# linnanwang/FastGen

Hardware: AMD Instinct MI355X
Metric: images/sec at 4-step distilled (DMD2) sampling (higher is better)
Workload: dtype fp32 (tensors, accumulate) with split-bf16 x3 MFMA conv products; 1 GPU; EDM CIFAR-10 32x32 SongUNet (55.7M params) DMD2 4-step 'sde' sampling, batch=512 per GPU; global_batch=512, sample_steps=4, parallelism=replicas x1 (no data-path collective), graph=True

## Files before the change

### fastgen_amd/csrc/conv_ws3.hip

```cpp
#include "common.h"
#include "conv.h"

namespace {

constexpr int X3_NTHR = 768;
constexpr int X3_KC = 32;
constexpr int X3_PA = 16;
constexpr int X3_PLANE = 3072;
constexpr int X3_ABUF = 8 * X3_PLANE;
constexpr int X3_RING = 4;
constexpr int X3_HOFF = 128 * 512;
constexpr int X3_LDS = X3_HOFF + X3_RING * X3_ABUF;
constexpr int X3_TAPB = 2048;

template <int LOGW>
struct X3Geom {
    static constexpr int W = 1 << LOGW;
    static constexpr int TW = 16, TH = 8;
    static constexpr int IPT = LOGW == 3 ? 2 : 1;
    static constexpr int TCOLS = LOGW == 3 ? 1 : W / TW;
    static constexpr int TPI = LOGW == 3 ? 1 : (W / TH) * TCOLS;
    static constexpr int HW_ = LOGW == 3 ? 2 * W + 3 : TW + 2, HH_ = TH + 2;
    static constexpr int HALO_PIX = HW_ * HH_;
    static constexpr int RS = HW_ * X3_PA;
    static_assert(HALO_PIX * X3_PA <= X3_PLANE && HALO_PIX <= 192, "one halo plane; three producer passes of 64 pixels");
};

__device__ __forceinline__ void x3_barrier() {
    asm volatile("s_waitcnt lgkmcnt(0)\n\ts_barrier" ::: "memory");
}

struct X3Frag {
    bf16x8 hi, lo;
};

template <int RES, int LOGW, int PRO>
__global__ __launch_bounds__(X3_NTHR) void conv3_x3ws_kernel(const ConvArgs a, const int ntiles) {
    using G = X3Geom<LOGW>;
    constexpr bool SUB = RES == RES_SUBPIX;
    constexpr int NTAP = SUB ? 4 : 9;
    constexpr int RN = SUB ? 4 : 3;
    constexpr int NQ = 4 * NTAP;
    constexpr int X3_STEPB = NTAP * X3_TAPB;
    extern __shared__ __attribute__((aligned(16))) char smem[];
    char* const hbuf = smem;
    char* const ring = smem + X3_HOFF;

    const int tid = threadIdx.x;
    const int lane = tid & 63;
    const int wave = __builtin_amdgcn_readfirstlane(tid >> 6);
    const int Cin = a.C1 + a.C2;
    const int nchunk = Cin / X3_KC;
    const int G8 = (int)gridDim.x >> 3;
    const int wg = ((gridDim.x & 7) == 0) ? ((int)blockIdx.x & 7) * G8 + ((int)blockIdx.x >> 3) : (int)blockIdx.x;
    const int gstride = (int)gridDim.x;
    const int my_tiles = (ntiles - wg + gstride - 1) / gstride;
    const int S = my_tiles * nchunk;
    const int NSTEP = S + 3;
    const int H = SUB ? a.Hs : a.H;

    if (wave < 8) {
        const int grp = wave >> 2, wl = wave & 3;
        const int col = lane & 15, g4 = lane >> 4;
        const size_t wstride = (size_t)nchunk * NTAP * 1024;
        const __amdgpu_buffer_rsrc_t wrs = __builtin_amdgcn_make_buffer_rsrc(
            const_cast<__bf16*>(reinterpret_cast<const __bf16*>(a.wpack_ws) + (size_t)(grp * 8 + wl * 2) * wstride), 0, 0x7fffffff,
            0x00020000);
        const int wvoff = lane * 16;
        const int wsb = (int)(wstride * 2);
        const int wphb = SUB ? 16 * wsb : 0;
        int tcur = wg;
        auto load_w = [&](int byte_off) -> X3Frag {
            X3Frag f;
            f.hi = __builtin_bit_cast(bf16x8, __builtin_amdgcn_raw_buffer_load_b128(wrs, wvoff, byte_off, 0));
            f.lo = __builtin_bit_cast(bf16x8, __builtin_amdgcn_raw_buffer_load_b128(wrs, wvoff, byte_off + 1024, 0));
            return f;
        };
        X3Frag wq[RN][2];
#pragma unroll
        for (int j = 0; j < RN; ++j)
#pragma unroll
            for (int nt = 0; nt < 2; ++nt) wq[j][nt] = load_w((tcur & 3) * wphb + nt * wsb + j * X3_TAPB);

        f32x4 acc[8][2];
#pragma unroll
        for (int m = 0; m < 8; ++m)
#pragma unroll
            for (int nt = 0; nt < 2; ++nt) acc[m][nt] = f32x4{0.f, 0.f, 0.f, 0.f};

        const int lane_off = g4 * X3_PLANE + (col + ((G::IPT == 2 && col >= 8) ? 1 : 0)) * X3_PA;
        const int dl0 = col * 512 + ((8 * wl + ((g4) ^ (col & 7))) << 4);
        const int dl1 = col * 512 + ((8 * wl + ((4 + g4) ^ (col & 7))) << 4);

        x3_barrier();
        int c = 0;
        for (int s = 0; s < NSTEP; ++s) {
            const int ls = s - 2 * grp;
            if (ls >= 0 && ls < S) {
                const char* abase = ring + (ls & 3) * X3_ABUF + lane_off + (SUB ? ((tcur >> 1) & 1) * G::RS + (tcur & 1) * X3_PA : 0);
                const int cn = (c + 1 == nchunk) ? 0 : c + 1;
                const int tnext = cn == 0 ? tcur + gstride : tcur;
                const int wcur = (tcur & 3) * wphb + c * X3_STEPB;
                const int wnxt = (ls + 1 < S) ? (tnext & 3) * wphb + cn * X3_STEPB : wcur;
                auto read_x = [&](int q, X3Frag (&xf)[2]) {
                    const int tap = q >> 2, m0 = 2 * (q & 3);
                    const int off = ((SUB ? tap >> 1 : tap / 3) + m0) * G::RS + (SUB ? tap & 1 : tap % 3) * X3_PA;
#pragma unroll
                    for (int m = 0; m < 2; ++m) {
                        xf[m].hi = *reinterpret_cast<const bf16x8*>(abase + off + m * G::RS);
                        xf[m].lo = *reinterpret_cast<const bf16x8*>(abase + off + m * G::RS + 4 * X3_PLANE);
                    }
                };
                auto mma12 = [&](int q, const X3Frag (&xf)[2]) {
                    const int tap = q >> 2, m0 = 2 * (q & 3);
                    const X3Frag(&wf)[2] = wq[tap % RN];
#pragma unroll
                    for (int m = 0; m < 2; ++m)
#pragma unroll
                        for (int nt = 0; nt < 2; ++nt)
                            acc[m0 + m][nt] = __builtin_amdgcn_mfma_f32_16x16x32_bf16(wf[nt].hi, xf[m].lo, acc[m0 + m][nt], 0, 0, 0);
#pragma unroll
                    for (int m = 0; m < 2; ++m)
#pragma unroll
                        for (int nt = 0; nt < 2; ++nt)
                            acc[m0 + m][nt] = __builtin_amdgcn_mfma_f32_16x16x32_bf16(wf[nt].lo, xf[m].hi, acc[m0 + m][nt], 0, 0, 0);
#pragma unroll
                    for (int m = 0; m < 2; ++m)
#pragma unroll
                        for (int nt = 0; nt < 2; ++nt)
                            acc[m0 + m][nt] = __builtin_amdgcn_mfma_f32_16x16x32_bf16(wf[nt].hi, xf[m].hi, acc[m0 + m][nt], 0, 0, 0);
                    if ((q & 3) != 3) return;
                    const int pn = (tap + RN < NTAP) ? wcur + (tap + RN) * X3_TAPB : wnxt + (tap + RN - NTAP) * X3_TAPB;
#pragma unroll
                    for (int nt = 0; nt < 2; ++nt) wq[tap % RN][nt] = load_w(pn + nt * wsb);
                };
                X3Frag x0[2], x1[2];
                read_x(0, x0);
#pragma unroll
                for (int q = 0; q < NQ; q += 2) {
                    read_x(q + 1, x1);
                    __builtin_amdgcn_sched_barrier(0);
                    mma12(q, x0);
                    __builtin_amdgcn_sched_barrier(0);
                    if (q + 2 < NQ) read_x(q + 2, x0);
                    __builtin_amdgcn_sched_barrier(0);
                    mma12(q + 1, x1);
                    __builtin_amdgcn_sched_barrier(0);
                }
                if (c + 1 == nchunk) {
#pragma unroll
                    for (int m = 0; m < 8; ++m) {
                        *reinterpret_cast<f32x4*>(hbuf + m * 8192 + dl0) = acc[m][0];
                        *reinterpret_cast<f32x4*>(hbuf + m * 8192 + dl1) = acc[m][1];
                        acc[m][0] = f32x4{0.f, 0.f, 0.f, 0.f};
                        acc[m][1] = f32x4{0.f, 0.f, 0.f, 0.f};
                    }
                }
                c = cn;
                tcur = tnext;
            }
            x3_barrier();
        }
        return;
    }

    const int ptid = tid - 512;
    const int pw = wave - 8;
    const int oct = ptid & 3;
    const float* src1 = reinterpret_cast<const float*>(a.src1);
    const float* src2 = reinterpret_cast<const float*>(a.src2);
    int hdy[3], hdx[3], hlds[3];
    bool third;
    const int pslot = ptid >> 2;
    const int pimg = (G::IPT == 2 && pslot >= 30) ? 1 : 0;
#pragma unroll
    for (int i = 0; i < 3; ++i) {
        int hy, hx;
        if (G::IPT == 2) {
            const int l = pimg ? min(pslot - 30 + 34 * i, 99) : pslot + 30 * i;
            hy = pimg ? l / 10 : l / 9;
            hx = pimg ? 9 + (l - hy * 10) : l - hy * 9;
            third = pimg ? pslot - 30 + 68 < 100 : true;
        } else {
            const int hq = min(pslot + 64 * i, G::HALO_PIX - 1);
            hy = hq / G::HW_;
            hx = hq - hy * G::HW_;
            third = pslot + 128 < G::HALO_PIX;
        }
        hdy[i] = hy - 1;
        hdx[i] = hx - 1 - pimg * (G::W + 1);
        hlds[i] = oct * X3_PLANE + hy * G::RS + hx * X3_PA;
    }

    auto tile_coord = [&](int t, int& n, int& slot, int& row0, int& col0) {
        if (SUB) t >>= 2;
        n = t * G::IPT / G::TPI;
        slot = t - n * G::TPI / G::IPT;
        row0 = (slot / G::TCOLS) * G::TH;
        col0 = (slot % G::TCOLS) * G::TW;
    };

    struct Staged {
        f32x4 raw[3][2];
        float2 ab[8];
    };
    unsigned off1[3], off2[3];
    bool valid[3];
    const float2* abn = a.ab;
    auto tile_setup = [&](int t) __attribute__((always_inline)) {
        int n, slot, row0, col0;
        tile_coord(t, n, slot, row0, col0);
        bool in_batch = true;
        if (G::IPT == 2) {
            n += pimg;
            in_batch = n < a.B;
            n = min(n, a.B - 1);
        }
#pragma unroll
        for (int i = 0; i < 3; ++i) {
            const int y = row0 + hdy[i], x = col0 + hdx[i];
            valid[i] = (y >= 0) && (y < H) && (x >= 0) && (x < G::W) && (i < 2 || third) && in_batch;
            const int yc = min(max(y, 0), H - 1), xc = min(max(x, 0), G::W - 1);
            const int sy = (RES == RES_UP) ? (yc >> 1) : yc, sx = (RES == RES_UP) ? (xc >> 1) : xc;
            const unsigned pix = (unsigned)((n * a.Hs + sy) * a.Ws + sx);
            off1[i] = (pix * (unsigned)a.C1 + oct * 8) * 4u;
            off2[i] = (pix * (unsigned)a.C2 + oct * 8) * 4u;
        }
        abn = a.ab + (size_t)n * Cin;
    };
    auto stage_load = [&](Staged& st, int t, int c32) __attribute__((always_inline)) {
        if (c32 == 0) tile_setup(t);
        const bool first = c32 * X3_KC < a.C1;
        const char* base = first ? reinterpret_cast<const char*>(src1) + c32 * (X3_KC * 4)
                                 : reinterpret_cast<const char*>(src2) + (c32 * X3_KC - a.C1) * 4;
#pragma unroll
        for (int i = 0; i < 3; ++i) {
            const char* p = base + (first ? off1[i] : off2[i]);
            st.raw[i][0] = *reinterpret_cast<const f32x4*>(p);
            st.raw[i][1] = *reinterpret_cast<const f32x4*>(p + 16);
        }
        if (PRO == PRO_NONE) return;
        const float2* p = abn + c32 * X3_KC + oct * 8;
#pragma unroll
        for (int j = 0; j < 8; j += 2) {
            const f32x4 q = *reinterpret_cast<const f32x4*>(p + j);
            st.ab[j] = make_float2(q[0], q[1]);
            st.ab[j + 1] = make_float2(q[2], q[3]);
        }
    };
    auto stage_store = [&](const Staged& st, char* abuf) __attribute__((always_inline)) {
#pragma unroll
        for (int i = 0; i < 3; ++i) {
            float v[8];
#pragma unroll
            for (int j = 0; j < 8; ++j) {
                v[j] = st.raw[i][j >> 2][j & 3];
                if (PRO != PRO_NONE) v[j] = silu_f<true>(fmaf(v[j], st.ab[j].x, st.ab[j].y));
            }
            bf16x8 hi, lo;
            split8(v, hi, lo);
            typedef __attribute__((ext_vector_type(4))) unsigned u32x4;
            u32x4 wh = __builtin_bit_cast(u32x4, hi), wl_ = __builtin_bit_cast(u32x4, lo);
#pragma unroll
            for (int j = 0; j < 4; ++j) {
                wh[j] = valid[i] ? wh[j] : 0u;
                wl_[j] = valid[i] ? wl_[j] : 0u;
            }
            if (i < 2 || third) {
                *reinterpret_cast<u32x4*>(abuf + hlds[i]) = wh;
                *reinterpret_cast<u32x4*>(abuf + hlds[i] + 4 * X3_PLANE) = wl_;
            }
        }
    };

    const int chq = lane & 31, psub = lane >> 5;
    float* const out = reinterpret_cast<float*>(a.out);
    const float* const resid = reinterpret_cast<const float*>(a.resid);
    const bool has_resid = __builtin_amdgcn_readfirstlane(resid != nullptr);
    auto retire_half = [&](int t, int half) __attribute__((always_inline)) {
        int n, slot, row0, col0;
        tile_coord(t, n, slot, row0, col0);
        const int co = half * 128 + chq * 4;
        const int nimg = G::IPT == 2 ? min(2, a.B - n) : 1;
        f32x4 radd[G::IPT];
#pragma unroll
        for (int k = 0; k < G::IPT; ++k) {
            radd[k] = f32x4{0.f, 0.f, 0.f, 0.f};
            if (a.bias) radd[k] = *reinterpret_cast<const f32x4*>(a.bias + co);
            const int nk = G::IPT == 2 ? min(n + k, a.B - 1) : n;
            if (a.temb) radd[k] += *reinterpret_cast<const f32x4*>(a.temb + (size_t)nk * a.temb_stride + co);
            radd[k] *= a.scale;
        }
        constexpr int OW = SUB ? 2 * G::W : G::W, OST = SUB ? 2 : 1;
        const int ph = t & 3;
        const size_t tb = SUB ? (((size_t)n * (2 * H) + 2 * row0 + (ph >> 1)) * OW + 2 * col0 + (ph & 1)) * 256 + co
                              : (((size_t)n * H + row0) * G::W + col0) * 256 + co;
        const int rs = (SUB || G::IPT == 2) ? 0 : a.rshift;
        const size_t rtb = (SUB || G::IPT == 2) ? tb : (((size_t)n * (H >> rs) + (row0 >> rs)) * (G::W >> rs) + (col0 >> rs)) * 256 + co;
        float ssum[G::IPT] = {}, ssq[G::IPT] = {};
#pragma unroll 1
        for (int grp8 = 0; grp8 < 2; ++grp8) {
            f32x4 rr[8], dv[8];
            unsigned go[8];
#pragma unroll
            for (int j = 0; j < 8; ++j) {
                const int px = pw * 32 + 2 * (grp8 * 8 + j) + psub;
                unsigned rgo;
                if (G::IPT == 2) {
                    go[j] = (unsigned)((((j >> 2) * OW + OST * (px >> 4)) * OW + OST * (px & 7)) * 256);
                    rgo = go[j];
                } else {
                    go[j] = (unsigned)((OST * (px >> 4) * OW + OST * (px & 15)) * 256);
                    rgo = SUB ? go[j] : (unsigned)((((px >> 4) >> rs) * (G::W >> rs) + ((px & 15) >> rs)) * 256);
                }
                rr[j] = f32x4{0.f, 0.f, 0.f, 0.f};
                if (has_resid && (G::IPT == 1 || (j >> 2) < nimg)) rr[j] = *reinterpret_cast<const f32x4*>(resid + rtb + rgo);
                dv[j] = *reinterpret_cast<const f32x4*>(hbuf + px * 512 + ((chq ^ (px & 7)) << 4));
            }
#pragma unroll
            for (int j = 0; j < 8; ++j) {
                const int k = G::IPT == 2 ? j >> 2 : 0;
                if (G::IPT == 2 && k >= nimg) continue;
                f32x4 v;
#pragma unroll
                for (int e = 0; e < 4; ++e) v[e] = fmaf(dv[j][e], a.scale, radd[k][e]);
                if (has_resid) {
#pragma unroll
                    for (int e = 0; e < 4; ++e) v[e] = fmaf(rr[j][e], a.scale, v[e]);
                }
                *reinterpret_cast<f32x4*>(out + tb + go[j]) = v;
                ssum[k] += (v[0] + v[1]) + (v[2] + v[3]);
                ssq[k] += (v[0] * v[0] + v[1] * v[1]) + (v[2] * v[2] + v[3] * v[3]);
            }
        }
#pragma unroll
        for (int k = 0; k < G::IPT; ++k) {
            ssum[k] += __shfl_xor(ssum[k], 32);
            ssq[k] += __shfl_xor(ssq[k], 32);
            const size_t sl = SUB ? ((size_t)(n + k) * G::TPI + slot) * 4 + ph : (size_t)(n + k) * G::TPI + slot;
            if (a.stats && psub == 0 && k < nimg) a.stats[(sl * 4 + pw) * 64 + half * 32 + chq] = make_float2(ssum[k], ssq[k]);
        }
    };

    auto advance = [&](int& t, int& cc) {
        if (++cc == nchunk) {
            cc = 0;
            t += gstride;
        }
    };
    Staged st;
    int t1 = wg, c1 = 0;
    stage_load(st, t1, c1);
    stage_store(st, ring);
    advance(t1, c1);
    x3_barrier();
    int sa = 0;
    for (int s = 0; s < NSTEP; ++s) {
        const bool more = s + 1 < S;
        if (more) stage_load(st, t1, c1);
        if (sa == 0 && s >= nchunk && s <= S) retire_half(wg + (s / nchunk - 1) * gstride, 0);
        if (sa == 2 % nchunk && s - 2 >= nchunk && s - 2 <= S && (s - 2) % nchunk == 0) retire_half(wg + ((s - 2) / nchunk - 1) * gstride, 1);
        if (more) {
            stage_store(st, ring + ((s + 1) & 3) * X3_ABUF);
            advance(t1, c1);
        }
        if (++sa == nchunk) sa = 0;
        x3_barrier();
    }
}

__global__ void pack_conv_weights_x3ws_kernel(const float* __restrict__ w, __bf16* __restrict__ out, int cout, int cin) {
    const size_t total = (size_t)cout * cin * 9;
    const int nstep = cin / X3_KC;
    for (size_t idx = (size_t)blockIdx.x * blockDim.x + threadIdx.x; idx < total; idx += (size_t)gridDim.x * blockDim.x) {
        size_t t = idx;
        const int j = t % 8; t /= 8;
        const int lane = t % 64; t /= 64;
        const int tap = t % 9; t /= 9;
        const int step = t % nstep; t /= nstep;
        const int n16 = (int)t;
        const int co = n16 * 16 + (lane & 15);
        const int ci = step * X3_KC + 8 * (lane >> 4) + j;
        const float v = w[((size_t)co * cin + ci) * 9 + tap];
        const __bf16 hi = (__bf16)v;
        const size_t o = (idx / 512) * 1024 + (idx % 512);
        out[o] = hi;
        out[o + 512] = (__bf16)(v - (float)hi);
    }
}

__global__ void pack_conv_weights_x3sub_kernel(const float* __restrict__ w, __bf16* __restrict__ out, int cout, int cin) {
    const size_t total = (size_t)16 * cout * cin;
    const int nstep = cin / X3_KC, ng = cout / 16;
    for (size_t idx = (size_t)blockIdx.x * blockDim.x + threadIdx.x; idx < total; idx += (size_t)gridDim.x * blockDim.x) {
        size_t t = idx;
        const int j = t % 8; t /= 8;
        const int lane = t % 64; t /= 64;
        const int tap = t % 4; t /= 4;
        const int step = t % nstep; t /= nstep;
        const int n16 = t % ng; t /= ng;
        const int py = (int)t >> 1, px = (int)t & 1, ty = tap >> 1, tx = tap & 1;
        const int co = n16 * 16 + (lane & 15);
        const int ci = step * X3_KC + 8 * (lane >> 4) + j;
        const int ky0 = py ? 2 * ty : ty, ky1 = py ? ty + 1 : 2 * ty;
        const int kx0 = px ? 2 * tx : tx, kx1 = px ? tx + 1 : 2 * tx;
        const float* wp = w + ((size_t)co * cin + ci) * 9;
        float v = 0.f;
        for (int ky = ky0; ky <= ky1; ++ky)
            for (int kx = kx0; kx <= kx1; ++kx) v += wp[ky * 3 + kx];
        const __bf16 hi = (__bf16)v;
        const size_t o = (idx / 512) * 1024 + (idx % 512);
        out[o] = hi;
        out[o + 512] = (__bf16)(v - (float)hi);
    }
}

int g_x3_cus[16] = {};

template <int RES, int LOGW, int PRO>
int launch_x3_one(const ConvArgs& a, hipStream_t stream, bool prepare_only) {
    using G = X3Geom<LOGW>;
    auto kern = conv3_x3ws_kernel<RES, LOGW, PRO>;
    int dev = 0;
    if (hipGetDevice(&dev) != hipSuccess || dev < 0 || dev >= 16) return (int)hipErrorInvalidDevice;
    static bool attr_done[16] = {};
    if (!attr_done[dev]) {
        hipError_t e = hipFuncSetAttribute(reinterpret_cast<const void*>(kern), hipFuncAttributeMaxDynamicSharedMemorySize, X3_LDS);
        if (e != hipSuccess) return (int)e;
        attr_done[dev] = true;
    }
    if (!g_x3_cus[dev]) {
        int n = 0;
        if (hipDeviceGetAttribute(&n, hipDeviceAttributeMultiprocessorCount, dev) != hipSuccess || n <= 0) return (int)hipErrorUnknown;
        g_x3_cus[dev] = n;
    }
    if (prepare_only) return 0;
    const int ntiles = (a.B * G::TPI + G::IPT - 1) / G::IPT * (RES == RES_SUBPIX ? 4 : 1);
    const int grid = ntiles < g_x3_cus[dev] ? ntiles : g_x3_cus[dev];
    hipLaunchKernelGGL(kern, dim3(grid), dim3(X3_NTHR), X3_LDS, stream, a, ntiles);
    return (int)hipGetLastError();
}

}

int conv_x3ws_stat_slots(int W, int res) {
    if (res == RES_SUBPIX) return (W == 32 ? X3Geom<4>::TPI : X3Geom<3>::TPI) * 16;
    return (W == 32 ? X3Geom<5>::TPI : W == 16 ? X3Geom<4>::TPI : X3Geom<3>::TPI) * 4;
}

bool conv_x3ws_shape_ok(int cout, int cin, int res) {
    return cout == 256 && (res == 32 || res == 16 || res == 8) && (cin % X3_KC) == 0 && cin / X3_KC >= 4;
}

bool conv_x3ws_supported(int ks, int pro, int res, int outmode, const ConvArgs& a) {
    const int cin = a.C1 + a.C2;
    const size_t src_bytes = (size_t)a.B * a.Hs * a.Ws * (size_t)(a.C1 > a.C2 ? a.C1 : a.C2) * 4;
    if (src_bytes >= (1ull << 32)) return false;
    if (res == RES_SUBPIX)
        return ks == 3 && outmode == OUT_NHWC && pro == PRO_GN_SILU && a.ab && a.H == a.W && a.Hs == a.Ws && a.H == 2 * a.Hs && (a.Ws == 16 || a.Ws == 8) &&
               conv_x3ws_shape_ok(a.Cout, cin, a.Ws) && (a.C1 % X3_KC) == 0 && a.wpack_ws && !a.rshift;
    if (ks != 3 || outmode != OUT_NHWC || a.H != a.W || !conv_x3ws_shape_ok(a.Cout, cin, a.W) || (a.C1 % X3_KC) || !a.wpack_ws) return false;
    if (a.W == 8 && res != RES_NONE) return false;
    if (a.rshift && (a.rshift != 1 || !a.resid || a.W == 8 || res != RES_NONE)) return false;
    if (pro == PRO_NONE) return res == RES_NONE && a.Hs == a.H && a.Ws == a.W;
    return pro == PRO_GN_SILU && (res == RES_NONE || res == RES_UP) && a.ab != nullptr;
}

int launch_conv_x3ws(int res, const ConvArgs& a, hipStream_t stream, bool prepare_only, int pro) {
    if (res == RES_SUBPIX) {
        if (pro != PRO_GN_SILU || (a.Ws != 16 && a.Ws != 8)) return (int)hipErrorInvalidValue;
        return a.Ws == 16 ? launch_x3_one<RES_SUBPIX, 4, PRO_GN_SILU>(a, stream, prepare_only) : launch_x3_one<RES_SUBPIX, 3, PRO_GN_SILU>(a, stream, prepare_only);
    }
    if (pro == PRO_NONE || a.W == 8) {
        if (res != RES_NONE) return (int)hipErrorInvalidValue;
        if (a.W == 8)
            return pro == PRO_NONE ? launch_x3_one<RES_NONE, 3, PRO_NONE>(a, stream, prepare_only)
                                   : launch_x3_one<RES_NONE, 3, PRO_GN_SILU>(a, stream, prepare_only);
        return a.W == 32 ? launch_x3_one<RES_NONE, 5, PRO_NONE>(a, stream, prepare_only) : launch_x3_one<RES_NONE, 4, PRO_NONE>(a, stream, prepare_only);
    }
    if (a.W == 32)
        return res == RES_UP ? launch_x3_one<RES_UP, 5, PRO_GN_SILU>(a, stream, prepare_only) : launch_x3_one<RES_NONE, 5, PRO_GN_SILU>(a, stream, prepare_only);
    return res == RES_UP ? launch_x3_one<RES_UP, 4, PRO_GN_SILU>(a, stream, prepare_only) : launch_x3_one<RES_NONE, 4, PRO_GN_SILU>(a, stream, prepare_only);
}

int launch_pack_conv_weights_x3ws(const float* w_oihw, void* wpack_ws, int cout, int cin, hipStream_t stream) {
    const size_t total = (size_t)cout * cin * 9;
    const int grid = (int)((total + 255) / 256 < 4096 ? (total + 255) / 256 : 4096);
    hipLaunchKernelGGL(pack_conv_weights_x3ws_kernel, dim3(grid), dim3(256), 0, stream, w_oihw, (__bf16*)wpack_ws, cout, cin);
    return (int)hipGetLastError();
}

int launch_pack_conv_weights_x3sub(const float* w_oihw, void* wpack_sub, int cout, int cin, hipStream_t stream) {
    const size_t total = (size_t)16 * cout * cin;
    const int grid = (int)((total + 255) / 256 < 4096 ? (total + 255) / 256 : 4096);
    hipLaunchKernelGGL(pack_conv_weights_x3sub_kernel, dim3(grid), dim3(256), 0, stream, w_oihw, (__bf16*)wpack_sub, cout, cin);
    return (int)hipGetLastError();
}
```

Measured before the change: 2792 img/s.

## Add lockstep single-tile variant of x3 warp-specialized conv kernel

When every workgroup owns at most one tile (ntiles <= grid), a LOCK variant runs both MFMA consumer groups in the same step instead of staggering group 1 by two steps. This shortens the pipeline from S+3 to S+1 steps, cutting drain latency. Group 1's accumulators go into free ring slots rather than the shared hbuf, so both halves can be retired together at the end. It adds a template variant and an environment toggle, at the cost of losing the producer/consumer stagger and possibly raising LDS-port contention.

Measured after the change: 2791 img/s. No clear change (-0.0%).

```diff
diff --git a/fastgen_amd/csrc/conv_ws3.hip b/fastgen_amd/csrc/conv_ws3.hip
--- a/fastgen_amd/csrc/conv_ws3.hip
+++ b/fastgen_amd/csrc/conv_ws3.hip
@@ -30,11 +30,16 @@
     asm volatile("s_waitcnt lgkmcnt(0)\n\ts_barrier" ::: "memory");
 }
 
+__device__ __forceinline__ int x3_lock_chunk(int m, int cur) {
+    const int j = (m * 11) >> 5;
+    return (j + (j >= cur ? 1 : 0)) * X3_ABUF + (m - 3 * j) * 8192;
+}
+
 struct X3Frag {
     bf16x8 hi, lo;
 };
 
-template <int RES, int LOGW, int PRO>
+template <int RES, int LOGW, int PRO, bool LOCK>
 __global__ __launch_bounds__(X3_NTHR) void conv3_x3ws_kernel(const ConvArgs a, const int ntiles) {
     using G = X3Geom<LOGW>;
     constexpr bool SUB = RES == RES_SUBPIX;
@@ -56,7 +61,8 @@
     const int gstride = (int)gridDim.x;
     const int my_tiles = (ntiles - wg + gstride - 1) / gstride;
     const int S = my_tiles * nchunk;
-    const int NSTEP = S + 3;
+    const int NSTEP = LOCK ? S + 1 : S + 3;
+    const int lock_cur = (S - 1) & 3;
     const int H = SUB ? a.Hs : a.H;
 
     if (wave < 8) {
@@ -95,7 +101,7 @@
         x3_barrier();
         int c = 0;
         for (int s = 0; s < NSTEP; ++s) {
-            const int ls = s - 2 * grp;
+            const int ls = LOCK ? s : s - 2 * grp;
             if (ls >= 0 && ls < S) {
                 const char* abase = ring + (ls & 3) * X3_ABUF + lane_off + (SUB ? ((tcur >> 1) & 1) * G::RS + (tcur & 1) * X3_PA : 0);
                 const int cn = (c + 1 == nchunk) ? 0 : c + 1;
@@ -148,10 +154,13 @@
                     __builtin_amdgcn_sched_barrier(0);
                 }
                 if (c + 1 == nchunk) {
+                    int cur = lock_cur;
+                    if (LOCK) asm volatile("" : "+s"(cur));
 #pragma unroll
                     for (int m = 0; m < 8; ++m) {
-                        *reinterpret_cast<f32x4*>(hbuf + m * 8192 + dl0) = acc[m][0];
-                        *reinterpret_cast<f32x4*>(hbuf + m * 8192 + dl1) = acc[m][1];
+                        char* const hb = (LOCK && grp) ? ring + x3_lock_chunk(m, cur) : hbuf + m * 8192;
+                        *reinterpret_cast<f32x4*>(hb + dl0) = acc[m][0];
+                        *reinterpret_cast<f32x4*>(hb + dl1) = acc[m][1];
                         acc[m][0] = f32x4{0.f, 0.f, 0.f, 0.f};
                         acc[m][1] = f32x4{0.f, 0.f, 0.f, 0.f};
                     }
@@ -277,7 +286,7 @@
     float* const out = reinterpret_cast<float*>(a.out);
     const float* const resid = reinterpret_cast<const float*>(a.resid);
     const bool has_resid = __builtin_amdgcn_readfirstlane(resid != nullptr);
-    auto retire_half = [&](int t, int half) __attribute__((always_inline)) {
+    auto retire_half = [&](int t, int half, const char* base, bool from_ring) __attribute__((always_inline)) {
         int n, slot, row0, col0;
         tile_coord(t, n, slot, row0, col0);
         const int co = half * 128 + chq * 4;
@@ -302,6 +311,7 @@
         for (int grp8 = 0; grp8 < 2; ++grp8) {
             f32x4 rr[8], dv[8];
             unsigned go[8];
+            const int cb = (LOCK && from_ring) ? x3_lock_chunk(2 * pw + grp8, lock_cur) - (2 * pw + grp8) * 8192 : 0;
 #pragma unroll
             for (int j = 0; j < 8; ++j) {
                 const int px = pw * 32 + 2 * (grp8 * 8 + j) + psub;
@@ -315,7 +325,7 @@
                 }
                 rr[j] = f32x4{0.f, 0.f, 0.f, 0.f};
                 if (has_resid && (G::IPT == 1 || (j >> 2) < nimg)) rr[j] = *reinterpret_cast<const f32x4*>(resid + rtb + rgo);
-                dv[j] = *reinterpret_cast<const f32x4*>(hbuf + px * 512 + ((chq ^ (px & 7)) << 4));
+                dv[j] = *reinterpret_cast<const f32x4*>(base + (LOCK ? cb : 0) + px * 512 + ((chq ^ (px & 7)) << 4));
             }
 #pragma unroll
             for (int j = 0; j < 8; ++j) {
@@ -357,9 +367,20 @@
     int sa = 0;
     for (int s = 0; s < NSTEP; ++s) {
         const bool more = s + 1 < S;
-        if (more) stage_load(st, t1, c1);
-        if (sa == 0 && s >= nchunk && s <= S) retire_half(wg + (s / nchunk - 1) * gstride, 0);
-        if (sa == 2 % nchunk && s - 2 >= nchunk && s - 2 <= S && (s - 2) % nchunk == 0) retire_half(wg + ((s - 2) / nchunk - 1) * gstride, 1);
+        if (more) {
+            if (LOCK) __builtin_assume(c1 != 0);
+            stage_load(st, t1, c1);
+        }
+        if (LOCK) {
+            if (s == S) {
+#pragma unroll 1
+                for (int half = 0; half < 2; ++half) retire_half(wg, half, half ? ring : hbuf, half != 0);
+            }
+        } else {
+            if (sa == 0 && s >= nchunk && s <= S) retire_half(wg + (s / nchunk - 1) * gstride, 0, hbuf, false);
+            if (sa == 2 % nchunk && s - 2 >= nchunk && s - 2 <= S && (s - 2) % nchunk == 0)
+                retire_half(wg + ((s - 2) / nchunk - 1) * gstride, 1, hbuf, false);
+        }
         if (more) {
             stage_store(st, ring + ((s + 1) & 3) * X3_ABUF);
             advance(t1, c1);
@@ -417,18 +438,32 @@
 
 int g_x3_cus[16] = {};
 
+bool x3_lockstep_enabled() {
+    static const bool on = [] {
+        const char* e = getenv("FASTGEN_AMD_CONV_LOCKSTEP");
+        return !(e && e[0] == '0');
+    }();
+    return on;
+}
+
+template <int RES, int LOGW, int PRO, bool LOCK>
+int x3_set_lds(int dev) {
+    static bool attr_done[16] = {};
+    if (attr_done[dev]) return 0;
+    hipError_t e = hipFuncSetAttribute(reinterpret_cast<const void*>(conv3_x3ws_kernel<RES, LOGW, PRO, LOCK>),
+                                       hipFuncAttributeMaxDynamicSharedMemorySize, X3_LDS);
+    if (e != hipSuccess) return (int)e;
+    attr_done[dev] = true;
+    return 0;
+}
+
 template <int RES, int LOGW, int PRO>
 int launch_x3_one(const ConvArgs& a, hipStream_t stream, bool prepare_only) {
     using G = X3Geom<LOGW>;
-    auto kern = conv3_x3ws_kernel<RES, LOGW, PRO>;
     int dev = 0;
     if (hipGetDevice(&dev) != hipSuccess || dev < 0 || dev >= 16) return (int)hipErrorInvalidDevice;
-    static bool attr_done[16] = {};
-    if (!attr_done[dev]) {
-        hipError_t e = hipFuncSetAttribute(reinterpret_cast<const void*>(kern), hipFuncAttributeMaxDynamicSharedMemorySize, X3_LDS);
-        if (e != hipSuccess) return (int)e;
-        attr_done[dev] = true;
-    }
+    if (int rc = x3_set_lds<RES, LOGW, PRO, false>(dev)) return rc;
+    if (int rc = x3_set_lds<RES, LOGW, PRO, true>(dev)) return rc;
     if (!g_x3_cus[dev]) {
         int n = 0;
         if (hipDeviceGetAttribute(&n, hipDeviceAttributeMultiprocessorCount, dev) != hipSuccess || n <= 0) return (int)hipErrorUnknown;
@@ -437,7 +472,10 @@
     if (prepare_only) return 0;
     const int ntiles = (a.B * G::TPI + G::IPT - 1) / G::IPT * (RES == RES_SUBPIX ? 4 : 1);
     const int grid = ntiles < g_x3_cus[dev] ? ntiles : g_x3_cus[dev];
-    hipLaunchKernelGGL(kern, dim3(grid), dim3(X3_NTHR), X3_LDS, stream, a, ntiles);
+    if (ntiles <= grid && x3_lockstep_enabled())
+        hipLaunchKernelGGL((conv3_x3ws_kernel<RES, LOGW, PRO, true>), dim3(grid), dim3(X3_NTHR), X3_LDS, stream, a, ntiles);
+    else
+        hipLaunchKernelGGL((conv3_x3ws_kernel<RES, LOGW, PRO, false>), dim3(grid), dim3(X3_NTHR), X3_LDS, stream, a, ntiles);
     return (int)hipGetLastError();
 }
 
```
